# mozilla/mozjpeg

Measured on AMD Instinct MI355X. Metric: Mpixels/s encode (4K RGB q75 trellis) at 1/2/4/8 GPUs; bit-exact vs cjpeg, higher is better.
Workload: dtype u8/int16 (+f32 trellis costs); 1 GPU; 3840x2160 synthetic RGB, q75 4:2:0 baseline, trellis+deringing+optimal Huffman (cjpeg -quality 75 -baseline); config_key=metric, frames_per_encode_call=96, distinct_frames=96, batches_in_flight=2, input=resident in HBM, output=complete JPEG files in HBM, parallelism=images sharded, 1 process per GPU, no collective

## Files before the change

### include/mozjpeg_hip.h

```cpp
#ifndef MOZJPEG_HIP_H
#define MOZJPEG_HIP_H

#include <stddef.h>
#include <stdint.h>

#ifdef __cplusplus
extern "C" {
#endif

#define MJH_MAX_COMPS 4
#define MJH_MAX_SCANS 64

#define MJH_OK            0
#define MJH_EINVAL       -1
#define MJH_EUNSUPPORTED -2
#define MJH_EHIP         -3
#define MJH_ENOMEM       -4
#define MJH_ETOOSMALL    -5

#define MJH_PROFILE_MAX_COMPRESSION 0x5D083AAD
#define MJH_PROFILE_FASTEST         0x2AEA5CB4

typedef struct {
  int comps_in_scan;
// ... 212 lines not shown
  int raw_coefs;
} mjh_decode_opts;
void mjh_decode_opts_defaults(mjh_decode_opts *o);
int mjh_decode_host(mjh_encoder *e, const void *const jpegs[], const size_t sizes[], int n, const mjh_decode_opts *opts);
int mjh_decode_wait(mjh_encoder *e);
int mjh_get_pixels(mjh_encoder *e, int i, void *dst, size_t row_pitch);
int mjh_get_pixels_device(mjh_encoder *e, void **d_base, size_t *row_pitch, size_t *image_stride);
int mjh_get_plane(mjh_encoder *e, int i, int comp, void *dst, size_t row_pitch, int width, int height);
int mjh_get_planes_device(mjh_encoder *e, int comp, void **d_base, size_t *row_pitch, size_t *image_stride, int *width, int *height);
int mjh_get_coefs_device(mjh_encoder *e, int comp, void **d_base, size_t *image_stride, int *blocks_per_row, int *height_in_blocks, int *width_in_blocks);
int mjh_get_coefs(mjh_encoder *e, int i, int comp, void *dst, size_t dst_blocks_per_row);
int mjh_get_coefs_ms(mjh_encoder *e, float *ms);
int mjh_decode_stats(mjh_encoder *e, int *width, int *height, int *pixel_size, float ms[2]);

int mjh_enc_onepass_stats(mjh_encoder *e, int *enabled, unsigned long long *long_blocks, unsigned long long *big_groups);
int mjh_get_dc_path(mjh_encoder *e, int *path);

int mjh_get_jpeg_size(mjh_encoder *e, int i, size_t *size);
int mjh_get_jpeg(mjh_encoder *e, int i, void *dst, size_t cap, size_t *size);
int mjh_get_output_device(mjh_encoder *e, void **d_base, size_t *stride, void **d_sizes);

int mjh_get_scan_table(mjh_encoder *e, int image, int scan, int tblno, uint8_t bits[17], uint8_t vals[256]);

enum {
  MJH_TAP_PLANE = 1,
  MJH_TAP_COEF_UQ = 2,
  MJH_TAP_COEF_Q = 3,
  MJH_TAP_COEF_Q0 = 4,
  MJH_TAP_HUFF_BITS = 5,
  MJH_TAP_HUFF_VALS = 6,
// ... 25 lines not shown
```

### mozjpeg_amd/__init__.py

```python
import ctypes as C
import os

import numpy as np

_HERE = os.path.dirname(os.path.abspath(__file__))
LIB_PATH = os.environ.get("MOZJPEG_AMD_LIB") or os.path.join(_HERE, "libmozjpeg_hip.so")

MAX_COMPS, MAX_SCANS = 4, 64
PROFILE_MAX_COMPRESSION = 0x5D083AAD
PROFILE_FASTEST = 0x2AEA5CB4
COLOR_YCC, COLOR_NONE, COLOR_YCC_IN = 0, 1, 2
CS_GRAYSCALE, CS_RGB, CS_YCBCR = 1, 2, 3
CS_CMYK, CS_YCCK = 4, 5
CS_RGB565 = 16
OK, EINVAL, EUNSUPPORTED, EHIP, ENOMEM, ETOOSMALL = 0, -1, -2, -3, -4, -5
TAP_PLANE, TAP_COEF_UQ, TAP_COEF_Q, TAP_COEF_Q0, TAP_HUFF_BITS, TAP_HUFF_VALS, TAP_PROG_SCAN_US, TAP_LL_COUNTS = 1, 2, 3, 4, 5, 6, 7, 8


class MjhError(RuntimeError):
    def __init__(self, code, msg):
        super().__init__("mozjpeg_hip error %d: %s" % (code, msg))
        self.code = code


# ... 174 lines not shown
            L.mjh_get_pixels_device.argtypes = [C.c_void_p, C.POINTER(C.c_void_p), C.POINTER(C.c_size_t), C.POINTER(C.c_size_t)]
            L.mjh_decode_stats.argtypes = [C.c_void_p, C.POINTER(C.c_int), C.POINTER(C.c_int), C.POINTER(C.c_int), C.POINTER(C.c_float)]
            L.mjh_decode_wait.argtypes = [C.c_void_p]
            L.mjh_get_plane.argtypes = [C.c_void_p, C.c_int, C.c_int, C.c_void_p, C.c_size_t, C.c_int, C.c_int]
            L.mjh_get_planes_device.argtypes = [C.c_void_p, C.c_int, C.POINTER(C.c_void_p), C.POINTER(C.c_size_t), C.POINTER(C.c_size_t),
                                                C.POINTER(C.c_int), C.POINTER(C.c_int)]
            L.mjh_transcode_batch_size.argtypes = [C.c_void_p]
        if hasattr(L, "mjh_get_coefs"):
            L.mjh_get_coefs.argtypes = [C.c_void_p, C.c_int, C.c_int, C.c_void_p, C.c_size_t]
            L.mjh_get_coefs_device.argtypes = [C.c_void_p, C.c_int, C.POINTER(C.c_void_p), C.POINTER(C.c_size_t)] + [C.POINTER(C.c_int)] * 3
            L.mjh_get_coefs_ms.argtypes = [C.c_void_p, C.POINTER(C.c_float)]
        if hasattr(L, "mjh_get_dc_path"):
            L.mjh_get_dc_path.argtypes = [C.c_void_p, C.POINTER(C.c_int)]
        if hasattr(L, "mjh_enc_onepass_stats"):
            L.mjh_enc_onepass_stats.argtypes = [C.c_void_p, C.POINTER(C.c_int), C.POINTER(C.c_ulonglong), C.POINTER(C.c_ulonglong)]
        _lib = L
    return _lib


def _chk(rc):
    if rc != 0:
        raise MjhError(rc, lib().mjh_last_error().decode())


def make_params(width, height, *, quality=75, baseline=False, revert=False, optimize=False,
                notrellis=False, notrellis_dc=False, noovershoot=False, sample=(2, 2), gray=False,
                grayin=False, quant_table=-1, lambda1=None, lambda2=None, restart=None,
                progressive=False, fastcrush=False, precision=8, trellis_loops=1, smooth=0, rgb=False,
                dc_scan_opt=None, dc_ver_weight=None, use_scans_in_trellis=False, trellis_freq_split=0,
                trellis_eob_opt=False, trellis_q_opt=False, arithmetic=False, arith_cond=None, scans=None, gray_sample=None, yccin=False, dct=None,
# ... 657 lines not shown

    def transcode_stats(self):
        a, b, c, ms = C.c_int(), C.c_int(), C.c_int(), (C.c_float * 4)()
        _chk(lib().mjh_transcode_stats(self._h, C.byref(a), C.byref(b), C.byref(c), ms))
        phases = dict(zip(("sync", "prefix", "store", "dc"), [float(x) for x in ms]))
        x = C.c_float()
        if hasattr(lib(), "mjh_get_coefs_ms") and lib().mjh_get_coefs_ms(self._h, C.byref(x)) == OK:
            phases["export"] = float(x.value)
        return dict(subseq=a.value, rounds=b.value, host_syncs=c.value, ms=phases)

    def enc_onepass_stats(self):
        on, a, b = C.c_int(), C.c_ulonglong(), C.c_ulonglong()
        _chk(lib().mjh_enc_onepass_stats(self._h, C.byref(on), C.byref(a), C.byref(b)))
        return dict(enabled=bool(on.value), long_blocks=a.value, big_groups=b.value)

    def dc_path(self):
        v = C.c_int()
        _chk(lib().mjh_get_dc_path(self._h, C.byref(v)))
        return (None, "lane", "dc3", "dc2", "speculative")[v.value]

    def transcode_host(self, files, errors="raise", **transform):
        n = len(files)
        if transform:
            self.set_transform(transform_spec(**transform))
        try:
            self.submit_transcode(files)
            return [self.get_jpeg(i) for i in range(n)]
        except MjhError:
            if errors != "return":
                raise
# ... 160 lines not shown
```

### mozjpeg_amd/csrc/mjh_encoder.cpp

```cpp
#include <hip/hip_runtime.h>

#include <math.h>
#include <stdarg.h>
#include <stdio.h>
#include <stdlib.h>
#include <string.h>

#include <array>
#include <atomic>
#include <condition_variable>
#include <functional>
#include <mutex>
#include <string>
#include <thread>
#include <memory>
#include <chrono>
#include <vector>

#include "../../include/mozjpeg_hip.h"
#include "mjh_internal.h"
#include "mjh_launch.h"
#include "mjh_lossless.h"
#include "mjh_decode.h"
#include "mjh_idct.h"
// ... 290 lines not shown
  void *d_prog_chunks = nullptr;
  int chunks_per_scan = 0;
  MjhProgPE pe{};
  PList pl_trellis[2]{}, pl_phase[4]{}, pl_trellis_c[2][4]{};
  int nphases = 0;
  unsigned *d_pool = nullptr; size_t pool_words = 0;
  uint8_t *d_outpool = nullptr; size_t outpool_bytes = 0;
  uint8_t *d_frame_hdr = nullptr; int frame_hdr_len = 0, file_hdr_len = 0;
  uint16_t *d_len16 = nullptr;
  unsigned *d_off32 = nullptr, *d_sums = nullptr, *d_totals = nullptr, *d_ffsums = nullptr, *d_fftotals = nullptr;
  unsigned *d_stream = nullptr;
  size_t stream_words = 0;
  int enc_onepass = 1;
  unsigned *d_pack = nullptr;
  size_t pack_words = 0;
  unsigned *d_enc_slow = nullptr;
  int chunks = 0, ff_chunks = 0;
  uint8_t *d_out = nullptr;
  size_t out_stride = 0;
  unsigned *d_sizes = nullptr;
  void *d_meta = nullptr;
  uint8_t *d_prefix = nullptr, *d_sos = nullptr;
  int prefix_len = 0, sos_len = 0;
  struct SeqScan { int ncomp; int comp[4]; int sos_off, sos_len; int dht_slots[8], dht_ids[8], ndht; int ri, nseg; };
  std::vector<SeqScan> seq_scans;
  int dht_slots[8] = { 0, 0, 0, 0, 0, 0, 0, 0 }, dht_ids[8] = { 0, 0, 0, 0, 0, 0, 0, 0 }, ndht = 0;
  bool debug_taps = false;
  int dc_chain_v = 1;
  int sof_hv0 = 0;
  bool fdct_div_zero = false;
// ... 545 lines not shown
{
  if (hipStreamSynchronize(a) != hipSuccess || hipStreamSynchronize(b) != hipSuccess) return -1;
  int votes = 0;
  for (int rep = 0; rep < 3; rep++) {
    const auto t0 = std::chrono::steady_clock::now();
    mjh_launch_spin(15000ull, a);
    mjh_launch_spin(15000ull, b);
    if (hipStreamSynchronize(a) != hipSuccess || hipStreamSynchronize(b) != hipSuccess) return -1;
    const double us = std::chrono::duration<double, std::micro>(std::chrono::steady_clock::now() - t0).count();
    votes += us < 240.0;
  }
  return votes >= 2;
}

static thread_local bool g_create_twin = false;
static thread_local int g_twin_onepass = 1;
static thread_local int g_twin_dc_lanes = 0, g_twin_dc_lanes_set = 0;
static thread_local hipStream_t g_twin_avoid[2] = { nullptr, nullptr };

static hipError_t make_streams(mjh_encoder *e)
{
#define STREAMCHK(x) do { const hipError_t r_ = (x); if (r_ != hipSuccess) return r_; } while (0)
  if (e->high_priority_streams) {
    std::vector<hipStream_t> made;
    for (int tries = 0; tries < 12 && !e->side_stream; tries++) {
      hipStream_t c = nullptr;
      STREAMCHK(hipStreamCreateWithFlags(&c, hipStreamNonBlocking));
      made.push_back(c);
      bool free_queue = true;
      for (hipStream_t other : { g_twin_avoid[0], g_twin_avoid[1], e->stream })
// ... 140 lines not shown
  if (const char *v = getenv("MJH_SMALL_BATCH")) e->small_batch = (size_t)atoll(v);
  if (const char *v = getenv("MJH_TRELLIS_CHUNKS")) { e->trellis_chunks = atoi(v); if (e->trellis_chunks < 0 || e->trellis_chunks > 4) e->trellis_chunks = 0; }
  for (int i = 0; i < 4; i++) HIPCHK_E(hipEventCreateWithFlags(&e->ev_chunk[i], hipEventDisableTiming));
  if (const char *v = getenv("MJH_DC_LATE")) { e->dc_late = atoi(v); if (e->dc_late < 0 || e->dc_late > 2) e->dc_late = 1; }
  if (g_create_twin) { e->dc_lanes = g_twin_dc_lanes; e->dc_lanes_set = g_twin_dc_lanes_set; }
  else if (const char *v = getenv("MJH_DC_LANES")) { e->dc_lanes = atoi(v); if (e->dc_lanes < 0) e->dc_lanes = 0; e->dc_lanes_set = 1; }
  e->dc_window_ok = 1;
  for (int i = 0; i < C.ncomp; i++) if (p->quantval[p->quant_tbl_no[i]][0] < 5) e->dc_window_ok = 0;
  if (const char *v = getenv("MJH_DC_SPEC")) e->dc_spec = atoi(v);
  if (const char *v = getenv("MJH_DECODE_SUBSEQ")) { e->dec_subseq = atoi(v); if (e->dec_subseq < 0 || (e->dec_subseq > 0 && e->dec_subseq < 16)) e->dec_subseq = 16; }
  HIPCHK_E(mjh_dmalloc((void **)&e->d_len16, B * (size_t)C.total_mcu_blocks * 2));
  HIPCHK_E(mjh_dmalloc((void **)&e->d_off32, B * (size_t)C.total_mcu_blocks * 4));
  e->chunks = (C.total_mcu_blocks + 2047) / 2048;
  if (g_create_twin) e->enc_onepass = g_twin_onepass;
  else if (const char *v = getenv("MJH_ENC_ONEPASS")) e->enc_onepass = atoi(v) != 0;
  if (e->enc_onepass) {
    e->pack_words = mjh_encode_pack_words(C);
    HIPCHK_E(mjh_dmalloc((void **)&e->d_pack, B * e->pack_words * 4));
    HIPCHK_E(mjh_dmalloc((void **)&e->d_enc_slow, 2 * sizeof(unsigned)));
    HIPCHK_E(hipMemset(e->d_enc_slow, 0, 2 * sizeof(unsigned)));
  }
  size_t words = (size_t)C.total_mcu_blocks * (C.precision == 12 ? 61 : 53) + 64;
  if (C.restart_interval) words += (size_t)(C.mcus_per_row * C.mcu_rows) / C.restart_interval + 1;
  if (words > (size_t)1 << 27) words = (size_t)1 << 27;
  e->stream_words = (words + 63) & ~(size_t)63;
  e->ff_chunks = (int)((e->stream_words + 2047) / 2048);
  HIPCHK_E(mjh_dmalloc((void **)&e->d_sums, B * (size_t)std::max(e->chunks, mjh_encode_segments(C)) * sizeof(unsigned)));
  HIPCHK_E(mjh_dmalloc((void **)&e->d_ffsums, B * e->ff_chunks * sizeof(unsigned)));
  HIPCHK_E(mjh_dmalloc((void **)&e->d_totals, B * sizeof(unsigned)));
  HIPCHK_E(mjh_dmalloc((void **)&e->d_fftotals, B * sizeof(unsigned)));
// ... 818 lines not shown
        int slots[8], ns = 0;
        for (int j = 0; j < q.ncomp; j++) {
          bool have_d = false, have_a = false;
          for (int t = 0; t < ns; t++) { have_d = have_d || slots[t] == v_dc[j]; have_a = have_a || slots[t] == v_ac[j]; }
          if (!have_d) slots[ns++] = v_dc[j];
          if (!have_a) slots[ns++] = v_ac[j];
        }
        mjh_launch_gen_tables(e->d_tabs, spi, slots, ns, n, s);
      }
      pr.mark("header");
      mjh_launch_header(si == 0 ? e->d_prefix : nullptr, si == 0 ? e->prefix_len : 0, e->d_sos + q.sos_off, q.sos_len, e->d_tabs, spi, q.dht_slots, q.dht_ids, q.ndht,
                        p.compress_profile != MJH_PROFILE_FASTEST, e->d_out, e->out_stride, e->d_meta, n, s, si == 0 ? nullptr : e->d_sizes);
      pr.mark("huff_encode");
      mjh_launch_encode(V, e->d_q, nzm, e->d_tabs, spi, v_dc, v_ac, e->d_len16, e->d_off32, e->d_sums, e->chunks, e->d_totals,
                        e->d_stream, e->stream_words, e->d_meta, e->d_seg_x, e->d_seg_E, e->d_seg_sums, e->d_seg_totals, e->d_mpos, q.nseg, n, s,
                        e->d_pack, e->pack_words, e->d_enc_slow);
      pr.mark("byte_stuff");
      mjh_launch_stuff(e->d_stream, e->stream_words, e->d_totals, e->d_ffsums, e->ff_chunks, e->d_fftotals, e->d_out, e->out_stride,
                       e->d_meta, e->d_sizes, e->d_mpos, q.nseg, n, s);
    }
  } else {
    if (p.optimize_coding) {
      pr.mark("stats_ac(final)");
      mjh_launch_stats_ac(C, e->d_q, nzm, e->d_tabs, spi, fin_ac, 1, n, s);
      if (!final_dc_counted) {
        pr.mark("stats_dc(final)");
        mjh_launch_stats_dc(C, e->d_q, e->d_tabs, spi, fin_dc, 1, zero4, n, s);
      }
      if (join_late) {
        pr.mark("join(trellis_dc)");
        HIPCHK(hipStreamWaitEvent(s, e->ev_join, 0));
      }
      pr.mark("gen_tables(final)");
      mjh_launch_gen_tables(e->d_tabs, spi, e->dht_slots, e->ndht, n, s);
    }
    if (before_output) HIPCHK(hipStreamWaitEvent(s, before_output, 0));
    pr.mark("header");
    mjh_launch_header(e->d_prefix, e->prefix_len, e->d_sos, e->sos_len, e->d_tabs, spi, e->dht_slots, e->dht_ids, e->ndht,
                      p.compress_profile != MJH_PROFILE_FASTEST, e->d_out, e->out_stride, e->d_meta, n, s);
    pr.mark("huff_encode");
    mjh_launch_encode(C, e->d_q, nzm, e->d_tabs, spi, fin_dc, fin_ac, e->d_len16, e->d_off32, e->d_sums, e->chunks, e->d_totals,
                      e->d_stream, e->stream_words, e->d_meta, e->d_seg_x, e->d_seg_E, e->d_seg_sums, e->d_seg_totals, e->d_mpos, e->nseg, n, s,
                      e->d_pack, e->pack_words, e->d_enc_slow);
    if (if_mode == 2) { HIPCHK(hipEventRecord(e->ev_done, s)); e->ev_done_set = true; }
    pr.mark("byte_stuff");
    mjh_launch_stuff(e->d_stream, e->stream_words, e->d_totals, e->d_ffsums, e->ff_chunks, e->d_fftotals, e->d_out, e->out_stride,
                     e->d_meta, e->d_sizes, e->d_mpos, e->nseg, n, s);
  }
  if (ext_qopt) {
    pr.mark("trellis_q_opt(DQT)");
    mjh_launch_qopt_fix(e->d_quant, e->d_out, e->out_stride, e->d_sizes, e->file_hdr_len, e->prefix_len - (10 + 3 * C.ncomp), e->dqt_tabs, e->dqt_ntab,
                        p.compress_profile != MJH_PROFILE_FASTEST, !e->progressive && C.precision == 8 && e->tbl_le1, n, s);
  }
  pr.mark(nullptr);
  pr.finish();
  if (peer && !(if_mode == 2 && e->ev_done_set)) { HIPCHK(hipEventRecord(e->ev_done, s)); e->ev_done_set = true; }
  HIPCHK(hipGetLastError());
  return MJH_OK;
// ... 3 lines not shown

static mjh_encoder *cur(mjh_encoder *e) { return e && e->last ? e->last : e; }

extern "C" int mjh_set_inflight(mjh_encoder *e, int batches)
{
  if (!e || batches < 1 || batches > 2) return fail(MJH_EINVAL, "batches in flight: 1 or 2");
  e->inflight = batches;
  return MJH_OK;
}

static int make_twin(mjh_encoder *e)
{
  mjh_encoder *t = nullptr;
  g_create_twin = true;
  g_twin_onepass = e->enc_onepass;
  g_twin_dc_lanes = e->dc_lanes; g_twin_dc_lanes_set = e->dc_lanes_set;
  g_twin_avoid[0] = e->stream; g_twin_avoid[1] = e->side_stream;
  const int rc = mjh_encoder_create(&e->p_created, e->max_batch, e->device, &t);
  g_create_twin = false;
  if (rc) return rc;
  t->owner = e;
  t->inflight = 1;
  t->profiling = e->profiling; t->prof_focus_name = e->prof_focus_name; t->prof_focus = e->prof_focus;
  e->twin = t;
  return MJH_OK;
}

static int wait_pending_pack(mjh_encoder *e, hipStream_t s)
{
  if (e->res_buf >= 0 && !e->res_waited[e->res_buf]) HIPCHK(hipStreamWaitEvent(s, e->ev_packed[e->res_buf], 0));
// ... 1968 lines not shown
  if (enabled) *enabled = e->enc_onepass;
  unsigned long long a = 0, b = 0;
  for (mjh_encoder *x : { e, e->twin }) {
    if (!x || !x->d_enc_slow) continue;
    unsigned h[2] = { 0, 0 };
    HIPCHK(hipSetDevice(x->device));
    HIPCHK(hipDeviceSynchronize());
    HIPCHK(hipMemcpy(h, x->d_enc_slow, sizeof(h), hipMemcpyDeviceToHost));
    a += h[0]; b += h[1];
  }
  if (long_blocks) *long_blocks = a;
  if (big_groups) *big_groups = b;
  return MJH_OK;
}

extern "C" int mjh_encoder_sync(mjh_encoder *e)
{
  if (!e) return fail(MJH_EINVAL, "null encoder");
  HIPCHK(hipSetDevice(e->device));
  HIPCHK(hipStreamSynchronize(e->last_stream ? e->last_stream : e->stream));
  if (e->twin) HIPCHK(hipStreamSynchronize(e->twin->last_stream ? e->twin->last_stream : e->twin->stream));
  return guard_verify();
}

static int fetch_sizes(mjh_encoder *e)
{
  if (e->sizes_valid) return MJH_OK;
  if (e->res_buf >= 0) {
    int rc = wait_results(e, e->res_buf);
    if (rc) return rc;
// ... 487 lines not shown
```

### mozjpeg_amd/csrc/mjh_kernels.hip

```cpp
#include <hip/hip_runtime.h>
#include <stdio.h>
#include <stdlib.h>
#include <stdint.h>
#include <type_traits>
#include <stdlib.h>
#include "mjh_internal.h"
#include "mjh_device.h"

#define WAVE 64

struct ZZTab { int v[64]; };
static constexpr ZZTab make_zz() {
  ZZTab t{};
  const int z[64] = {
    0,  1,  8, 16,  9,  2,  3, 10, 17, 24, 32, 25, 18, 11,  4,  5,
    12, 19, 26, 33, 40, 48, 41, 34, 27, 20, 13,  6,  7, 14, 21, 28,
    35, 42, 49, 56, 57, 50, 43, 36, 29, 22, 15, 23, 30, 37, 44, 51,
    58, 59, 52, 45, 38, 31, 39, 46, 53, 60, 61, 54, 47, 55, 62, 63 };
  for (int i = 0; i < 64; i++) t.v[i] = z[i];
  return t;
}
static constexpr ZZTab kZZ = make_zz();

#define FIXC(x) ((int)((x) * 65536.0 + 0.5))
// ... 647 lines not shown
  __syncthreads();
  const int c4 = (lane & 7) * 4;
#pragma unroll
  for (int i = 0; i < 8; i++) {
    const int b = i * 8 + (lane >> 3);
    const unsigned *t = tile + b * 33 + c4;
    if (d0 + b < ndst) *reinterpret_cast<uint4 *>(out + (size_t)(d0 + b) * 128 + (size_t)c4 * 4) = make_uint4(t[0], t[1], t[2], t[3]);
  }
}
template <class F>
__device__ __forceinline__ void for_each_nonzero(const int16_t *__restrict__ qb, size_t kstride, unsigned long long mask, bool active, F &&f)
{
  const int n = active ? __popcll(mask) : 0;
#pragma unroll 1
  for (int base = 0; base < 63; base += 8) {
    if (__builtin_amdgcn_ballot_w64(base < n) == 0ull) break;
    int v[8];
#pragma unroll
    for (int j = 0; j < 8; j++) v[j] = (base + j < n) ? (int)qb[(size_t)(base + j + 1) * kstride] : 0;
#pragma unroll
    for (int j = 0; j < 8; j++)
      if (base + j < n) {
        const int pos = __builtin_ctzll(mask);
        mask &= mask - 1ull;
        f(pos, v[j]);
      }
  }
}

#define STATS_AC_ITER 4
// ... 1092 lines not shown
  __device__ __forceinline__ MarkerCursor(const unsigned *m, int nmark) : mpos(m), n(nmark), idx(-1) {}
  __device__ __forceinline__ bool at(unsigned bytepos)
  {
    if (idx < 0) {
      int lo = 0, hi = n;
      while (lo < hi) { const int mid = (lo + hi) >> 1; if (mpos[mid] < bytepos) lo = mid + 1; else hi = mid; }
      idx = lo;
    }
    while (idx < n && mpos[idx] < bytepos) idx++;
    return idx < n && mpos[idx] == bytepos;
  }
};

#define ENCW_WIN 4096

template <bool COMPACT, class W>
__device__ __forceinline__ void enc_write_block(const MjhConst &C, const MjhComp &cc, W &bw, const unsigned *s_ac, const unsigned *s_dc,
                                                const int16_t *__restrict__ q, const unsigned long long *__restrict__ nzmask_img, int r, int c,
                                                int *dc_nbits = nullptr)
{
  const int dc = q[dc_source_block(cc, r, c)];
  int pr, pc, pred = 0;
  if (mcu_prev_block(C, cc, r, c, pr, pc)) pred = q[dc_source_block(cc, pr, pc)];
  {
    const int df = dc - pred;
    const int a = df < 0 ? -df : df;
    const int nb = bitlen((unsigned)a);
    if (dc_nbits) *dc_nbits = nb;
    const unsigned e = s_dc[nb];
    bw.put(e & 0xFFFF, (int)(e >> 16));
// ... 100 lines not shown
      bw.flush();
    };
    if (window) { BitSink<true> bw; bw.init(s_win, fo - (w0 << 5)); emit(bw, w0 << 5); }
    else { BitSink<false> bw; bw.init(g, fo); emit(bw, 0u); }
  }
  __syncthreads();
  if (window)
    for (unsigned i = tid; i < nw; i += 256) {
      const unsigned v = s_win[i];
      if (v == 0u) continue;
      if (i == 0u || i == nw - 1u) atomicOr(&g[w0 + i], v);
      else g[w0 + i] = v;
    }
}

#define ENCP_DEPTH 8
#define ENCP_WIN 2048

__device__ __forceinline__ void enc_load_tables(unsigned (*s_ac)[256], unsigned (*s_dc)[32], const MjhConst &C, const MjhHuffTable *__restrict__ tabs_img,
                                                const int4 &dc_slot_of_comp, const int4 &ac_slot_of_comp)
{
  const int tid = threadIdx.x;
  for (int ci = 0; ci < C.ncomp; ci++) {
    const int dslot = ci == 0 ? dc_slot_of_comp.x : ci == 1 ? dc_slot_of_comp.y : ci == 2 ? dc_slot_of_comp.z : dc_slot_of_comp.w;
    const int aslot = ci == 0 ? ac_slot_of_comp.x : ci == 1 ? ac_slot_of_comp.y : ci == 2 ? ac_slot_of_comp.z : ac_slot_of_comp.w;
    const MjhHuffTable *TD = tabs_img + dslot;
    const MjhHuffTable *TA = tabs_img + aslot;
    s_ac[ci][tid] = ((unsigned)TA->ehufsi[tid] << 16) | TA->ehufco[tid];
    if (tid < 32) s_dc[ci][tid] = tid < 16 ? ((unsigned)TD->ehufsi[tid] << 16) | TD->ehufco[tid] : 0u;
  }
}

__device__ __forceinline__ int enc_scan_position(const MjhConst &C, int p, int &r, int &c)
{
  const int mcu = p / C.blocks_per_mcu, bi = p - mcu * C.blocks_per_mcu;
  int comp = 0;
  for (int ci = 1; ci < C.ncomp; ci++) if (bi >= C.c[ci].mcu_blk0) comp = ci;
  const int h = C.c[comp].h, v = C.c[comp].v;
  const int local = bi - C.c[comp].mcu_blk0, yi = local / h, xi = local - yi * h;
  const int mrow = mcu / C.mcus_per_row, mcol = mcu - mrow * C.mcus_per_row;
  r = mrow * v + yi;
  c = mcol * h + xi;
  return comp;
}

template <bool COMPACT>
__global__ void __launch_bounds__(256)
k_enc_write_pack(MjhConst C, const int16_t *__restrict__ coef_q, const unsigned long long *__restrict__ nzmask, const MjhHuffTable *__restrict__ tabs,
                 int slots_per_image, int4 dc_slot_of_comp, int4 ac_slot_of_comp,
                 unsigned *__restrict__ pack, size_t pack_words_per_image, unsigned *__restrict__ sums, int segs_per_image,
                 MjhImageMeta *__restrict__ meta, unsigned *__restrict__ slow)
{
  __shared__ unsigned s_ac[MJH_MAXC][256];
  __shared__ unsigned s_dc[MJH_MAXC][32];
  __shared__ unsigned s_stage[ENCP_DEPTH * 256];
  __shared__ uint4 s_win4[ENCP_WIN / 4];
  __shared__ unsigned sh[8];
  unsigned *s_win = reinterpret_cast<unsigned *>(s_win4);
  const int img = blockIdx.y, tid = threadIdx.x;
  const int N = C.total_mcu_blocks, p = blockIdx.x * 256 + tid;
  enc_load_tables(s_ac, s_dc, C, tabs + (size_t)img * slots_per_image, dc_slot_of_comp, ac_slot_of_comp);
  for (int i = tid; i < ENCP_WIN / 4; i += 256) s_win4[i] = make_uint4(0u, 0u, 0u, 0u);
  __syncthreads();
  int r = 0, c = 0;
  const int comp = enc_scan_position(C, p < N ? p : 0, r, c);
  const MjhComp cc = C.c[comp];
  const int16_t *q = coef_q + (size_t)img * C.coefs_per_image + cc.coef_off;
  const unsigned long long *nzi = COMPACT ? nzmask + (size_t)img * C.total_real_blocks : nullptr;
  unsigned bits = 0;
  if (p < N) {
    MJH_DIVERGENT_SCOPE;
    StageSink<ENCP_DEPTH, 256> bw;
    bw.init(s_stage + tid);
    int nb = 0;
    enc_write_block<COMPACT>(C, cc, bw, s_ac[comp], s_dc[comp], q, nzi, r, c, &nb);
    bw.flush();
    bits = bw.bitpos();
    if (nb > (C.precision == 12 ? 15 : 11)) meta[img].bad_coef = 1u;
  }
  unsigned tot;
  const unsigned ex = block_excl_scan_256_1b(bits, sh, 0, &tot);
  if (tid == 0) sums[(size_t)img * segs_per_image + blockIdx.x] = tot;
  const unsigned nw = (tot + 31u) >> 5;
  if (nw > (unsigned)ENCP_WIN) {
    if (tid == 0) atomicAdd(&slow[1], 1u);
    return;
  }
  if (bits > ENCP_DEPTH * 32u) {
    MJH_DIVERGENT_SCOPE;
    atomicAdd(&slow[0], 1u);
    BitSink<true, false> bw;
    bw.init(s_win, ex);
    enc_write_block<COMPACT>(C, cc, bw, s_ac[comp], s_dc[comp], q, nzi, r, c);
    bw.flush();
  } else {
    const unsigned s = ex & 31u, w0 = ex >> 5, nsw = (bits + 31u) >> 5, ndw = (s + bits + 31u) >> 5;
    unsigned prev = 0u;
    for (unsigned k = 0; k < ndw; k++) {
      const unsigned cur = k < nsw ? s_stage[k * 256 + tid] : 0u;
      const unsigned v = funnel_shift(prev, cur, s);
      if (v) atomicOr(&s_win[w0 + k], v);
      prev = cur;
    }
  }
  __syncthreads();
  unsigned *g = pack + (size_t)img * pack_words_per_image + (size_t)blockIdx.x * ENCP_WIN;
  for (unsigned i = tid; i < nw; i += 256) g[i] = s_win[i];
}

__global__ void __launch_bounds__(256)
k_enc_write_place(const unsigned *__restrict__ pack, size_t pack_words_per_image, const unsigned *__restrict__ sums, int segs_per_image,
                  const unsigned *__restrict__ totals, unsigned *__restrict__ stream, size_t stream_words_per_image)
{
  const int img = blockIdx.y, lane = threadIdx.x & 63;
  const int seg = blockIdx.x * 4 + (threadIdx.x >> 6);
  if (seg >= segs_per_image) return;
  const unsigned total = totals[img];
  if (total == 0xFFFFFFFFu) return;
  const unsigned *sm = sums + (size_t)img * segs_per_image;
  const unsigned base = sm[seg], len = (seg + 1 < segs_per_image ? sm[seg + 1] : total) - base;
  const unsigned nsw = (len + 31u) >> 5;
  if (nsw > (unsigned)ENCP_WIN) return;
// ... 545 lines not shown
    return MJH_DC_PATH_LANE;
  }
  dim3 grid((chain1 - chain0 + 3) / 4, n);
  if (window_ok && C.delta_dc_weight <= 0.0f) {
    hipLaunchKernelGGL(k_trellis_dc3, grid, dim3(64), 0, s, C, Q, (const int16_t *)uq, (int16_t *)q, tabs, spi, make_int4(dc_slot[0], dc_slot[1], dc_slot[2], dc_slot[3]), lambda, (uint8_t *)back, chain0, chain1);
    return MJH_DC_PATH_DC3;
  }
  hipLaunchKernelGGL(k_trellis_dc2, grid, dim3(64), 0, s, C, Q, (const int16_t *)uq, (int16_t *)q, tabs, spi, make_int4(dc_slot[0], dc_slot[1], dc_slot[2], dc_slot[3]), lambda, (uint8_t *)back, chain0, chain1);
  return MJH_DC_PATH_DC2;
}

void mjh_launch_encode(const MjhConst &C, const void *q, const unsigned long long *nzmask, const MjhHuffTable *tabs, int spi, const int dc_slot[4], const int ac_slot[4],
                       void *len16, void *off32, unsigned *sums, int chunks_per_image, unsigned *totals,
                       unsigned *stream, size_t stream_words_per_image, void *meta,
                       unsigned *seg_x, unsigned *seg_E, unsigned *seg_sums, unsigned *seg_totals, unsigned *mpos, int nseg,
                       int n, hipStream_t s, unsigned *pack, size_t pack_words_per_image, unsigned *slow)
{
  const int4 ds = make_int4(dc_slot[0], dc_slot[1], dc_slot[2], dc_slot[3]);
  const int4 as = make_int4(ac_slot[0], ac_slot[1], ac_slot[2], ac_slot[3]);
  if (pack && C.restart_interval == 0) {
    const int segs = mjh_encode_segments(C);
    dim3 gridp(segs, n);
    if (nzmask) hipLaunchKernelGGL((k_enc_write_pack<true>), gridp, dim3(256), 0, s, C, (const int16_t *)q, nzmask, tabs, spi, ds, as, pack, pack_words_per_image, sums, segs,
                                   (MjhImageMeta *)meta, slow);
    else hipLaunchKernelGGL((k_enc_write_pack<false>), gridp, dim3(256), 0, s, C, (const int16_t *)q, nzmask, tabs, spi, ds, as, pack, pack_words_per_image, sums, segs,
                            (MjhImageMeta *)meta, slow);
    hipLaunchKernelGGL(k_scan_sums, dim3(n), dim3(256), 0, s, sums, segs, totals, (const unsigned *)nullptr);
    hipLaunchKernelGGL(k_zero_stream, dim3(64, n), dim3(256), 0, s, stream, stream_words_per_image, (const unsigned *)totals, (const unsigned *)nullptr);
    hipLaunchKernelGGL(k_enc_write_place, dim3((segs + 3) / 4, n), dim3(256), 0, s, (const unsigned *)pack, pack_words_per_image, (const unsigned *)sums, segs,
                       (const unsigned *)totals, stream, stream_words_per_image);
    dim3 gridb((segs + 255) / 256, n);
    if (nzmask) hipLaunchKernelGGL((k_enc_write_big<true>), gridb, dim3(256), 0, s, C, (const int16_t *)q, nzmask, tabs, spi, ds, as, (const unsigned *)sums, segs,
                                   (const unsigned *)totals, stream, stream_words_per_image);
    else hipLaunchKernelGGL((k_enc_write_big<false>), gridb, dim3(256), 0, s, C, (const int16_t *)q, nzmask, tabs, spi, ds, as, (const unsigned *)sums, segs,
                            (const unsigned *)totals, stream, stream_words_per_image);
    hipLaunchKernelGGL(k_finish_bits, dim3((n + 63) / 64), dim3(64), 0, s, totals, (const unsigned *)nullptr, stream, stream_words_per_image, (MjhImageMeta *)meta, n);
    return;
  }
  dim3 grid((max_padblk(C) + 255) / 256, C.ncomp, n);
  if (nzmask) hipLaunchKernelGGL((k_enc_len<true>), grid, dim3(256), 0, s, C, (const int16_t *)q, nzmask, tabs, spi, ds, as, (uint16_t *)len16, (MjhImageMeta *)meta);
  else hipLaunchKernelGGL((k_enc_len<false>), grid, dim3(256), 0, s, C, (const int16_t *)q, nzmask, tabs, spi, ds, as, (uint16_t *)len16, (MjhImageMeta *)meta);
// ... 59 lines not shown
```

### mozjpeg_amd/csrc/mjh_launch.h

```cpp
#ifndef MJH_LAUNCH_H
#define MJH_LAUNCH_H
#include <hip/hip_runtime.h>
#include "mjh_internal.h"

void mjh_launch_import_coefs(const MjhConst &C, const MjhCoefSrc &S, void *coef_q, void *meta, int n, hipStream_t s);
void mjh_launch_export_coefs(const MjhConst &C, const MjhCoefDst &D, const void *coef_q, const unsigned *status, int n, hipStream_t s);
void mjh_launch_import_planes(const MjhConst &C, const MjhPlaneSrc &S, void *planes, int n, hipStream_t s);
void mjh_launch_color(const MjhConst &C, const void *pix, size_t row_pitch, size_t img_stride, void *planes, int n, hipStream_t s);
void mjh_launch_dct(const MjhConst &C, const MjhQuant *Q, const void *planes, void *uq, void *q, float *lambda,
                    MjhHuffTable *stat_tabs, int spi, const int stat_slot[4], uint8_t *nq8, int n, hipStream_t s, int fastdiv = 0, int ifast = 0);
void mjh_launch_stats_ac(const MjhConst &C, const void *q, const unsigned long long *nzmask, MjhHuffTable *tabs, int spi, const int slot[4], int count_dummies, int n, hipStream_t s);
void mjh_launch_stats_dc(const MjhConst &C, const void *q, MjhHuffTable *tabs, int spi, const int slot[4], int mcu_order, const int comp_restart[4], int n, hipStream_t s);
void mjh_launch_gen_tables(MjhHuffTable *tabs, int spi, const int *slots, int nslots, int n, hipStream_t s);
void mjh_launch_trellis_ac(const MjhConst &C, const MjhQuant *Q, const void *uq, void *q, MjhHuffTable *tabs, int spi, const int ac_slot[4], const float *lambda,
                           unsigned *worklist, unsigned *worklist2, void *dense, unsigned dense_cap, int variant,
                           int Ss, int Se, void *eob_cost, int *eob_has, unsigned long long *nzmask, int qstride, int n, hipStream_t s,
                           uint8_t *nq8 = nullptr, int v3_passes = 0, int fastdiv = 0, hipEvent_t after_first_tier = nullptr, hipEvent_t after_first_tier2 = nullptr,
                           int chunks = 1, hipStream_t side = nullptr, hipEvent_t *ev_chunk = nullptr, int count_mask = 0);
void mjh_launch_trellis_eob_chain(const MjhConst &C, void *q, const MjhHuffTable *tabs, int spi, const int ac_slot[4], const void *eob_cost, const int *eob_has,
                                  int Ss, int Se, int n, hipStream_t s);
void mjh_launch_qopt_accumulate(const MjhConst &C, const void *uq, const void *q, void *sums, int n, hipStream_t s);
void mjh_launch_qopt_update(void *sums, MjhQuant *Q, int n, hipStream_t s);
void mjh_launch_qopt_fix(const MjhQuant *Q, void *out, size_t out_stride, unsigned *sizes, int dqt_start, int sof_off, const int *tabs, int ntab,
                         int multi, int baseline_capable, int n, hipStream_t s);
enum { MJH_DC_PATH_NONE = 0, MJH_DC_PATH_LANE = 1, MJH_DC_PATH_DC3 = 2, MJH_DC_PATH_DC2 = 3, MJH_DC_PATH_SPEC = 4 };
bool mjh_trellis_dc_lanes_ok(const MjhConst &C, int window_ok, int n, int lanes_min);
int mjh_launch_trellis_dc(const MjhConst &C, const MjhQuant *Q, const void *uq, void *q, const MjhHuffTable *tabs, int spi, const int dc_slot[4], const float *lambda, void *back, int n, hipStream_t s,
                          int window_ok = 0, int chain0 = 0, int chain1 = -1, int lanes_min = 0);
void mjh_launch_encode(const MjhConst &C, const void *q, const unsigned long long *nzmask, const MjhHuffTable *tabs, int spi, const int dc_slot[4], const int ac_slot[4],
                       void *len16, void *off32, unsigned *sums, int chunks_per_image, unsigned *totals,
                       unsigned *stream, size_t stream_words_per_image, void *meta,
                       unsigned *seg_x, unsigned *seg_E, unsigned *seg_sums, unsigned *seg_totals, unsigned *mpos, int nseg,
                       int n, hipStream_t s, unsigned *pack = nullptr, size_t pack_words_per_image = 0, unsigned *slow = nullptr);
int mjh_encode_segments(const MjhConst &C);
size_t mjh_encode_pack_words(const MjhConst &C);
void mjh_launch_header(const void *prefix, int prefix_len, const void *sos, int sos_len, const MjhHuffTable *tabs, int spi,
                       const int dht_slots[8], const int dht_ids[8], int ndht, int multi_dht, void *out, size_t out_stride, void *meta, int n, hipStream_t s, const unsigned *append_sizes = nullptr);
void mjh_launch_finish_bits(unsigned *totals, unsigned *stream, size_t stream_words_per_image, void *meta, int n, hipStream_t s);
void mjh_launch_stuff(const unsigned *stream, size_t stream_words_per_image, const unsigned *totals, unsigned *ffsums, int ff_chunks_per_image,
                      unsigned *ff_totals, void *out, size_t out_stride, void *meta, unsigned *sizes, const unsigned *mpos, int nseg, int n, hipStream_t s);
void mjh_launch_pack_results(const void *out, size_t out_stride, const unsigned *sizes, const void *meta, const void *prog_ctl, int n,
                             void *dst, size_t cap, void *table, hipStream_t s);
void mjh_launch_pack_results_spliced(const void *out, size_t out_stride, const unsigned *sizes, const void *meta, const void *prog_ctl, int n,
                                     const MjhSpliceFile *files, const MjhSpliceRun *runs, const void *tc, const void *icc, unsigned icc_len, unsigned hdr,
                                     void *dst, size_t cap, void *table, hipStream_t s);
void mjh_launch_spin(unsigned long long ticks_100mhz, hipStream_t s);
void mjh_launch_gen_tables_list(MjhHuffTable *tabs, int spi, const int *d_slots, int nslots, int n, hipStream_t s);
void mjh_launch_prog_reset(void *ctl, int nscans, int n, hipStream_t s);
// ... 25 lines not shown
```

Measured before the change: 159,100 Mpixels/s.

## Persist pack-encode blocks across segment groups with prefetch and division-free scan positions

Measured after the change: 164,300 Mpixels/s (median of 6 runs). 1.03x the previous value.

```diff
diff --git a/include/mozjpeg_hip.h b/include/mozjpeg_hip.h
--- a/include/mozjpeg_hip.h
+++ b/include/mozjpeg_hip.h
@@ -250,6 +250,7 @@
 int mjh_decode_stats(mjh_encoder *e, int *width, int *height, int *pixel_size, float ms[2]);
 
 int mjh_enc_onepass_stats(mjh_encoder *e, int *enabled, unsigned long long *long_blocks, unsigned long long *big_groups);
+int mjh_enc_pack_groups(mjh_encoder *e, int *groups, int *twin_groups);
 int mjh_get_dc_path(mjh_encoder *e, int *path);
 
 int mjh_get_jpeg_size(mjh_encoder *e, int i, size_t *size);
diff --git a/mozjpeg_amd/__init__.py b/mozjpeg_amd/__init__.py
--- a/mozjpeg_amd/__init__.py
+++ b/mozjpeg_amd/__init__.py
@@ -212,6 +212,9 @@
             L.mjh_get_dc_path.argtypes = [C.c_void_p, C.POINTER(C.c_int)]
         if hasattr(L, "mjh_enc_onepass_stats"):
             L.mjh_enc_onepass_stats.argtypes = [C.c_void_p, C.POINTER(C.c_int), C.POINTER(C.c_ulonglong), C.POINTER(C.c_ulonglong)]
+        if hasattr(L, "mjh_enc_pack_groups"):
+            L.mjh_enc_pack_groups.argtypes = [C.c_void_p, C.POINTER(C.c_int), C.POINTER(C.c_int)]
+            L.mjh_enc_scan_positions.argtypes = [C.c_int] + [C.POINTER(C.c_int)] * 4 + [C.c_int, C.POINTER(C.c_int), C.c_int, C.POINTER(C.c_int)]
         _lib = L
     return _lib
 
@@ -899,6 +902,11 @@
         _chk(lib().mjh_enc_onepass_stats(self._h, C.byref(on), C.byref(a), C.byref(b)))
         return dict(enabled=bool(on.value), long_blocks=a.value, big_groups=b.value)
 
+    def enc_pack_groups(self):
+        g, t = C.c_int(), C.c_int()
+        _chk(lib().mjh_enc_pack_groups(self._h, C.byref(g), C.byref(t)))
+        return g.value, (None if t.value < 0 else t.value)
+
     def dc_path(self):
         v = C.c_int()
         _chk(lib().mjh_get_dc_path(self._h, C.byref(v)))
diff --git a/mozjpeg_amd/csrc/mjh_encoder.cpp b/mozjpeg_amd/csrc/mjh_encoder.cpp
--- a/mozjpeg_amd/csrc/mjh_encoder.cpp
+++ b/mozjpeg_amd/csrc/mjh_encoder.cpp
@@ -328,6 +328,7 @@
   int enc_onepass = 1;
   unsigned *d_pack = nullptr;
   size_t pack_words = 0;
+  int encp_groups = MJH_ENCP_GROUPS_DEFAULT;
   unsigned *d_enc_slow = nullptr;
   int chunks = 0, ff_chunks = 0;
   uint8_t *d_out = nullptr;
@@ -903,6 +904,7 @@
 }
 
 static thread_local bool g_create_twin = false;
+static thread_local int g_twin_encp_groups = MJH_ENCP_GROUPS_DEFAULT;
 static thread_local int g_twin_onepass = 1;
 static thread_local int g_twin_dc_lanes = 0, g_twin_dc_lanes_set = 0;
 static thread_local hipStream_t g_twin_avoid[2] = { nullptr, nullptr };
@@ -1073,6 +1075,8 @@
   e->chunks = (C.total_mcu_blocks + 2047) / 2048;
   if (g_create_twin) e->enc_onepass = g_twin_onepass;
   else if (const char *v = getenv("MJH_ENC_ONEPASS")) e->enc_onepass = atoi(v) != 0;
+  if (g_create_twin) e->encp_groups = g_twin_encp_groups;
+  else if (const char *v = getenv("MJH_ENCP_GROUPS")) { e->encp_groups = atoi(v); if (e->encp_groups < 1 || e->encp_groups > 64) e->encp_groups = MJH_ENCP_GROUPS_DEFAULT; }
   if (e->enc_onepass) {
     e->pack_words = mjh_encode_pack_words(C);
     HIPCHK_E(mjh_dmalloc((void **)&e->d_pack, B * e->pack_words * 4));
@@ -1921,7 +1925,7 @@
       pr.mark("huff_encode");
       mjh_launch_encode(V, e->d_q, nzm, e->d_tabs, spi, v_dc, v_ac, e->d_len16, e->d_off32, e->d_sums, e->chunks, e->d_totals,
                         e->d_stream, e->stream_words, e->d_meta, e->d_seg_x, e->d_seg_E, e->d_seg_sums, e->d_seg_totals, e->d_mpos, q.nseg, n, s,
-                        e->d_pack, e->pack_words, e->d_enc_slow);
+                        e->d_pack, e->pack_words, e->d_enc_slow, e->encp_groups);
       pr.mark("byte_stuff");
       mjh_launch_stuff(e->d_stream, e->stream_words, e->d_totals, e->d_ffsums, e->ff_chunks, e->d_fftotals, e->d_out, e->out_stride,
                        e->d_meta, e->d_sizes, e->d_mpos, q.nseg, n, s);
@@ -1948,7 +1952,7 @@
     pr.mark("huff_encode");
     mjh_launch_encode(C, e->d_q, nzm, e->d_tabs, spi, fin_dc, fin_ac, e->d_len16, e->d_off32, e->d_sums, e->chunks, e->d_totals,
                       e->d_stream, e->stream_words, e->d_meta, e->d_seg_x, e->d_seg_E, e->d_seg_sums, e->d_seg_totals, e->d_mpos, e->nseg, n, s,
-                      e->d_pack, e->pack_words, e->d_enc_slow);
+                      e->d_pack, e->pack_words, e->d_enc_slow, e->encp_groups);
     if (if_mode == 2) { HIPCHK(hipEventRecord(e->ev_done, s)); e->ev_done_set = true; }
     pr.mark("byte_stuff");
     mjh_launch_stuff(e->d_stream, e->stream_words, e->d_totals, e->d_ffsums, e->ff_chunks, e->d_fftotals, e->d_out, e->out_stride,
@@ -1982,6 +1986,7 @@
   mjh_encoder *t = nullptr;
   g_create_twin = true;
   g_twin_onepass = e->enc_onepass;
+  g_twin_encp_groups = e->encp_groups;
   g_twin_dc_lanes = e->dc_lanes; g_twin_dc_lanes_set = e->dc_lanes_set;
   g_twin_avoid[0] = e->stream; g_twin_avoid[1] = e->side_stream;
   const int rc = mjh_encoder_create(&e->p_created, e->max_batch, e->device, &t);
@@ -3980,6 +3985,14 @@
   return MJH_OK;
 }
 
+extern "C" int mjh_enc_pack_groups(mjh_encoder *e, int *groups, int *twin_groups)
+{
+  if (!e) return fail(MJH_EINVAL, "null encoder");
+  if (groups) *groups = e->encp_groups;
+  if (twin_groups) *twin_groups = e->twin ? e->twin->encp_groups : -1;
+  return MJH_OK;
+}
+
 extern "C" int mjh_encoder_sync(mjh_encoder *e)
 {
   if (!e) return fail(MJH_EINVAL, "null encoder");
diff --git a/mozjpeg_amd/csrc/mjh_kernels.hip b/mozjpeg_amd/csrc/mjh_kernels.hip
--- a/mozjpeg_amd/csrc/mjh_kernels.hip
+++ b/mozjpeg_amd/csrc/mjh_kernels.hip
@@ -685,6 +685,33 @@
   const int n = active ? __popcll(mask) : 0;
 #pragma unroll 1
   for (int base = 0; base < 63; base += 8) {
+    if (__builtin_amdgcn_ballot_w64(base < n) == 0ull) break;
+    int v[8];
+#pragma unroll
+    for (int j = 0; j < 8; j++) v[j] = (base + j < n) ? (int)qb[(size_t)(base + j + 1) * kstride] : 0;
+#pragma unroll
+    for (int j = 0; j < 8; j++)
+      if (base + j < n) {
+        const int pos = __builtin_ctzll(mask);
+        mask &= mask - 1ull;
+        f(pos, v[j]);
+      }
+  }
+}
+
+template <class F>
+__device__ __forceinline__ void for_each_nonzero_from(const int *v0, const int16_t *__restrict__ qb, size_t kstride, unsigned long long mask, bool active, F &&f)
+{
+  const int n = active ? __popcll(mask) : 0;
+#pragma unroll
+  for (int j = 0; j < 8; j++)
+    if (j < n) {
+      const int pos = __builtin_ctzll(mask);
+      mask &= mask - 1ull;
+      f(pos, v0[j]);
+    }
+#pragma unroll 1
+  for (int base = 8; base < 63; base += 8) {
     if (__builtin_amdgcn_ballot_w64(base < n) == 0ull) break;
     int v[8];
 #pragma unroll
@@ -1807,6 +1834,62 @@
 
 #define ENCW_WIN 4096
 
+template <class W>
+__device__ __forceinline__ void enc_put_dc(W &bw, const unsigned *s_dc, int df, int *dc_nbits)
+{
+  const int a = df < 0 ? -df : df;
+  const int nb = bitlen((unsigned)a);
+  if (dc_nbits) *dc_nbits = nb;
+  const unsigned e = s_dc[nb];
+  bw.put(e & 0xFFFF, (int)(e >> 16));
+  if (nb) bw.put((unsigned)(df < 0 ? df - 1 : df), nb);
+}
+
+template <bool COMPACT, class W>
+__device__ __forceinline__ void enc_put_ac(int kstride, W &bw, const unsigned *s_ac, const int16_t *__restrict__ q, unsigned long long m, bool real, int b,
+                                           const int *v0 = nullptr)
+{
+  if (COMPACT) {
+    int prev = 0;
+    auto sym = [&](int pos, int v) {
+      int run = pos - prev - 1;
+      prev = pos;
+      while (run > 15) { const unsigned e = s_ac[0xF0]; bw.put(e & 0xFFFF, (int)(e >> 16)); run -= 16; }
+      const int a = v < 0 ? -v : v;
+      const int nbv = bitlen((unsigned)a);
+      const unsigned e = s_ac[(run << 4) + nbv];
+      bw.put_sym(e, (unsigned)(v < 0 ? v - 1 : v), nbv);
+    };
+    if (v0) for_each_nonzero_from(v0, q + b, (size_t)kstride, m, real, sym);
+    else for_each_nonzero(q + b, (size_t)kstride, m, real, sym);
+    if (!real || prev < 63) { const unsigned e = s_ac[0]; bw.put(e & 0xFFFF, (int)(e >> 16)); }
+  } else {
+    int x[64];
+#pragma unroll
+    for (int k = 1; k < 64; k++) x[k] = q[(size_t)k * kstride + b];
+    if (real) {
+      int run = 0;
+#pragma unroll
+      for (int k = 1; k < 64; k++) {
+        const int v = x[k];
+        if (v == 0) run++;
+        else {
+          while (run > 15) { const unsigned e = s_ac[0xF0]; bw.put(e & 0xFFFF, (int)(e >> 16)); run -= 16; }
+          const int a = v < 0 ? -v : v;
+          const int nb = bitlen((unsigned)a);
+          const unsigned e = s_ac[(run << 4) + nb];
+          bw.put_sym(e, (unsigned)(v < 0 ? v - 1 : v), nb);
+          run = 0;
+        }
+      }
+      if (run > 0) { const unsigned e = s_ac[0]; bw.put(e & 0xFFFF, (int)(e >> 16)); }
+    } else {
+      const unsigned e = s_ac[0];
+      bw.put(e & 0xFFFF, (int)(e >> 16));
+    }
+  }
+}
+
 template <bool COMPACT, class W>
 __device__ __forceinline__ void enc_write_block(const MjhConst &C, const MjhComp &cc, W &bw, const unsigned *s_ac, const unsigned *s_dc,
                                                 const int16_t *__restrict__ q, const unsigned long long *__restrict__ nzmask_img, int r, int c,
@@ -1937,7 +2020,14 @@
     }
 }
 
+#ifndef ENCP_DEPTH
 #define ENCP_DEPTH 8
+#endif
+#ifdef ENCP_MIN_WAVES
+#define ENCP_BOUNDS __launch_bounds__(256, ENCP_MIN_WAVES)
+#else
+#define ENCP_BOUNDS __launch_bounds__(256)
+#endif
 #define ENCP_WIN 2048
 
 __device__ __forceinline__ void enc_load_tables(unsigned (*s_ac)[256], unsigned (*s_dc)[32], const MjhConst &C, const MjhHuffTable *__restrict__ tabs_img,
@@ -1967,68 +2057,191 @@
   return comp;
 }
 
+__host__ __device__ __forceinline__ int udiv_m31(int n, unsigned m, unsigned s)
+{
+  return (int)((unsigned)(((unsigned long long)((unsigned)n << 1) * m) >> 32) >> s);
+}
+
+static void mjh_enc_div_magic(unsigned d, unsigned *m, unsigned *s)
+{
+  unsigned sh = 0;
+  while ((1u << sh) < d) sh++;
+  *m = (unsigned)((((unsigned long long)1 << (31 + sh)) + d - 1) / d);
+  *s = sh;
+}
+
+struct EncComp { int h, v, wib, hib, mcu_blk0, kstride; long long coef_off, blk_off; };
+__host__ __device__ __forceinline__ EncComp enc_comp(const MjhComp &m)
+{
+  EncComp e;
+  e.h = m.h; e.v = m.v; e.wib = m.wib; e.hib = m.hib; e.mcu_blk0 = m.mcu_blk0; e.kstride = m.kstride; e.coef_off = m.coef_off; e.blk_off = m.blk_off;
+  return e;
+}
+
+__host__ __device__ __forceinline__ int enc_dc_source(const EncComp &cc, int r, int c, int mcol)
+{
+  if (r >= cc.hib) { c = mcol * cc.h + cc.h - 1; r = cc.hib - 1; }
+  if (c > cc.wib - 1) c = cc.wib - 1;
+  return r * cc.wib + c;
+}
+
+__host__ __device__ __forceinline__ int enc_scan_position_nodiv(const MjhConst &C, const EncComp *cs, const uint4 &dv, int p, int &r, int &c, int &dc_blk, int &pred_blk)
+{
+  const int mcu = udiv_m31(p, dv.x, dv.y), bi = p - mcu * C.blocks_per_mcu;
+  int comp = 0;
+  for (int ci = 1; ci < C.ncomp; ci++) if (bi >= C.c[ci].mcu_blk0) comp = ci;
+  const EncComp cc = cs[comp];
+  const int h = cc.h, v = cc.v;
+  const int local = bi - cc.mcu_blk0;
+  const int yi = (local * (int)((0x10162040u >> (8 * (h - 1))) & 0xFFu)) >> 6, xi = local - yi * h;
+  const int mrow = udiv_m31(mcu, dv.z, dv.w), mcol = mcu - mrow * C.mcus_per_row;
+  r = mrow * v + yi;
+  c = mcol * h + xi;
+  dc_blk = enc_dc_source(cc, r, c, mcol);
+  int pr = r, pc = c - 1, pmcol = mcol;
+  bool has = true;
+  if (xi == 0) {
+    if (yi > 0) { pr = r - 1; pc = c + h - 1; }
+    else if (mcu == 0) has = false;
+    else {
+      const bool wrap = mcol == 0;
+      pmcol = wrap ? C.mcus_per_row - 1 : mcol - 1;
+      pr = (wrap ? mrow - 1 : mrow) * v + v - 1;
+      pc = pmcol * h + h - 1;
+    }
+  }
+  pred_blk = has ? enc_dc_source(cc, pr, pc, pmcol) : -1;
+  return comp;
+}
+
+extern "C" int mjh_enc_scan_positions(int ncomp, const int *h, const int *v, const int *wib, const int *hib, int mcus_per_row,
+                                      const int *p, int np, int *out)
+{
+  if (ncomp < 1 || ncomp > MJH_MAXC || mcus_per_row < 1) return -1;
+  MjhConst C{};
+  C.ncomp = ncomp;
+  C.mcus_per_row = mcus_per_row;
+  for (int i = 0; i < ncomp; i++) {
+    if (h[i] < 1 || h[i] > 4 || v[i] < 1 || v[i] > 4) return -1;
+    C.c[i].h = h[i]; C.c[i].v = v[i]; C.c[i].wib = wib[i]; C.c[i].hib = hib[i];
+    C.c[i].mcu_blk0 = C.blocks_per_mcu;
+    C.blocks_per_mcu += h[i] * v[i];
+  }
+  EncComp cs[MJH_MAXC];
+  for (int i = 0; i < ncomp; i++) cs[i] = enc_comp(C.c[i]);
+  uint4 dv;
+  mjh_enc_div_magic((unsigned)C.blocks_per_mcu, &dv.x, &dv.y);
+  mjh_enc_div_magic((unsigned)C.mcus_per_row, &dv.z, &dv.w);
+  for (int i = 0; i < np; i++) {
+    int *o = out + 5 * (size_t)i;
+    o[0] = enc_scan_position_nodiv(C, cs, dv, p[i], o[1], o[2], o[3], o[4]);
+  }
+  return 0;
+}
+
+#ifndef ENCP_AHEAD
+#define ENCP_AHEAD 1
+#endif
+#ifndef ENCP_EARLY
+#define ENCP_EARLY 1
+#endif
 template <bool COMPACT>
-__global__ void __launch_bounds__(256)
+__global__ void ENCP_BOUNDS
 k_enc_write_pack(MjhConst C, const int16_t *__restrict__ coef_q, const unsigned long long *__restrict__ nzmask, const MjhHuffTable *__restrict__ tabs,
                  int slots_per_image, int4 dc_slot_of_comp, int4 ac_slot_of_comp,
                  unsigned *__restrict__ pack, size_t pack_words_per_image, unsigned *__restrict__ sums, int segs_per_image,
-                 MjhImageMeta *__restrict__ meta, unsigned *__restrict__ slow)
+                 MjhImageMeta *__restrict__ meta, unsigned *__restrict__ slow, int groups, uint4 dv)
 {
   __shared__ unsigned s_ac[MJH_MAXC][256];
   __shared__ unsigned s_dc[MJH_MAXC][32];
   __shared__ unsigned s_stage[ENCP_DEPTH * 256];
   __shared__ uint4 s_win4[ENCP_WIN / 4];
   __shared__ unsigned sh[8];
+  __shared__ EncComp s_cc[MJH_MAXC];
   unsigned *s_win = reinterpret_cast<unsigned *>(s_win4);
+  constexpr bool AHEAD = COMPACT && ENCP_AHEAD;
   const int img = blockIdx.y, tid = threadIdx.x;
-  const int N = C.total_mcu_blocks, p = blockIdx.x * 256 + tid;
+  const int N = C.total_mcu_blocks;
+  if (tid < C.ncomp) s_cc[tid] = enc_comp(C.c[tid]);
+  if (AHEAD && ENCP_EARLY) __syncthreads();
+  const int16_t *qimg = coef_q + (size_t)img * C.coefs_per_image;
+  const unsigned long long *nzi = COMPACT ? nzmask + (size_t)img * C.total_real_blocks : nullptr;
+  const int max_nb = C.precision == 12 ? 15 : 11;
+  const int seg0 = blockIdx.x * groups, seg1 = min(seg0 + groups, segs_per_image);
+  struct Pos { int comp, b, df, kstride; bool real; const int16_t *q; unsigned long long m; int v0[8]; };
+  auto fetch = [&](int seg, Pos &P) {
+    const int p = seg * 256 + tid;
+    int r, c, dcb, pdb;
+    P.comp = enc_scan_position_nodiv(C, s_cc, dv, p < N ? p : 0, r, c, dcb, pdb);
+    const EncComp cc = s_cc[P.comp];
+    P.q = qimg + cc.coef_off;
+    P.real = r < cc.hib && c < cc.wib;
+    P.b = P.real ? r * cc.wib + c : 0;
+    P.kstride = cc.kstride;
+    P.m = 0ull;
+    if (COMPACT) P.m = nzi[cc.blk_off + P.b];
+    if (AHEAD) {
+#pragma unroll
+      for (int j = 0; j < 8; j++) P.v0[j] = (int)P.q[(size_t)(j + 1) * cc.kstride + P.b];
+    }
+    const int dc = P.q[dcb], pred = P.q[pdb < 0 ? dcb : pdb];
+    P.df = dc - (pdb < 0 ? 0 : pred);
+  };
+  Pos P;
+  if (AHEAD && ENCP_EARLY) fetch(seg0, P);
   enc_load_tables(s_ac, s_dc, C, tabs + (size_t)img * slots_per_image, dc_slot_of_comp, ac_slot_of_comp);
   for (int i = tid; i < ENCP_WIN / 4; i += 256) s_win4[i] = make_uint4(0u, 0u, 0u, 0u);
   __syncthreads();
-  int r = 0, c = 0;
-  const int comp = enc_scan_position(C, p < N ? p : 0, r, c);
-  const MjhComp cc = C.c[comp];
-  const int16_t *q = coef_q + (size_t)img * C.coefs_per_image + cc.coef_off;
-  const unsigned long long *nzi = COMPACT ? nzmask + (size_t)img * C.total_real_blocks : nullptr;
-  unsigned bits = 0;
-  if (p < N) {
-    MJH_DIVERGENT_SCOPE;
-    StageSink<ENCP_DEPTH, 256> bw;
-    bw.init(s_stage + tid);
-    int nb = 0;
-    enc_write_block<COMPACT>(C, cc, bw, s_ac[comp], s_dc[comp], q, nzi, r, c, &nb);
-    bw.flush();
-    bits = bw.bitpos();
-    if (nb > (C.precision == 12 ? 15 : 11)) meta[img].bad_coef = 1u;
-  }
-  unsigned tot;
-  const unsigned ex = block_excl_scan_256_1b(bits, sh, 0, &tot);
-  if (tid == 0) sums[(size_t)img * segs_per_image + blockIdx.x] = tot;
-  const unsigned nw = (tot + 31u) >> 5;
-  if (nw > (unsigned)ENCP_WIN) {
-    if (tid == 0) atomicAdd(&slow[1], 1u);
-    return;
-  }
-  if (bits > ENCP_DEPTH * 32u) {
-    MJH_DIVERGENT_SCOPE;
-    atomicAdd(&slow[0], 1u);
-    BitSink<true, false> bw;
-    bw.init(s_win, ex);
-    enc_write_block<COMPACT>(C, cc, bw, s_ac[comp], s_dc[comp], q, nzi, r, c);
-    bw.flush();
-  } else {
-    const unsigned s = ex & 31u, w0 = ex >> 5, nsw = (bits + 31u) >> 5, ndw = (s + bits + 31u) >> 5;
-    unsigned prev = 0u;
-    for (unsigned k = 0; k < ndw; k++) {
-      const unsigned cur = k < nsw ? s_stage[k * 256 + tid] : 0u;
-      const unsigned v = funnel_shift(prev, cur, s);
-      if (v) atomicOr(&s_win[w0 + k], v);
-      prev = cur;
-    }
-  }
-  __syncthreads();
-  unsigned *g = pack + (size_t)img * pack_words_per_image + (size_t)blockIdx.x * ENCP_WIN;
-  for (unsigned i = tid; i < nw; i += 256) g[i] = s_win[i];
+  if (AHEAD && !ENCP_EARLY) fetch(seg0, P);
+#pragma unroll 1
+  for (int seg = seg0; seg < seg1; seg++) {
+    if (!AHEAD) fetch(seg, P);
+    const int p = seg * 256 + tid, comp = P.comp, kstride = P.kstride;
+    unsigned bits = 0;
+    if (p < N) {
+      MJH_DIVERGENT_SCOPE;
+      StageSink<ENCP_DEPTH, 256> bw;
+      bw.init(s_stage + tid);
+      int nb = 0;
+      enc_put_dc(bw, s_dc[comp], P.df, &nb);
+      enc_put_ac<COMPACT>(kstride, bw, s_ac[comp], P.q, P.m, P.real, P.b, AHEAD ? P.v0 : nullptr);
+      bw.flush();
+      bits = bw.bitpos();
+      if (nb > max_nb) meta[img].bad_coef = 1u;
+    }
+    if (AHEAD && seg + 1 < seg1) fetch(seg + 1, P);
+    unsigned tot;
+    const unsigned ex = block_excl_scan_256_1b(bits, sh, (seg - seg0) & 1, &tot);
+    if (tid == 0) sums[(size_t)img * segs_per_image + seg] = tot;
+    const unsigned nw = (tot + 31u) >> 5;
+    if (nw > (unsigned)ENCP_WIN) {
+      if (tid == 0) atomicAdd(&slow[1], 1u);
+      continue;
+    }
+    if (bits > ENCP_DEPTH * 32u) {
+      MJH_DIVERGENT_SCOPE;
+      atomicAdd(&slow[0], 1u);
+      Pos Q;
+      fetch(seg, Q);
+      BitSink<true, false> bw;
+      bw.init(s_win, ex);
+      enc_put_dc(bw, s_dc[comp], Q.df, nullptr);
+      enc_put_ac<COMPACT>(Q.kstride, bw, s_ac[comp], Q.q, Q.m, Q.real, Q.b);
+      bw.flush();
+    } else {
+      const unsigned s = ex & 31u, w0 = ex >> 5, nsw = (bits + 31u) >> 5, ndw = (s + bits + 31u) >> 5;
+      unsigned prev = 0u;
+      for (unsigned k = 0; k < ndw; k++) {
+        const unsigned cw = k < nsw ? s_stage[k * 256 + tid] : 0u;
+        const unsigned v = funnel_shift(prev, cw, s);
+        if (v) atomicOr(&s_win[w0 + k], v);
+        prev = cw;
+      }
+    }
+    __syncthreads();
+    uint4 *g = reinterpret_cast<uint4 *>(pack + (size_t)img * pack_words_per_image + (size_t)seg * ENCP_WIN);
+    for (unsigned i = tid; i < (nw + 3u) >> 2; i += 256) { g[i] = s_win4[i]; s_win4[i] = make_uint4(0u, 0u, 0u, 0u); }
+  }
 }
 
 __global__ void __launch_bounds__(256)
@@ -2604,17 +2817,21 @@
                        void *len16, void *off32, unsigned *sums, int chunks_per_image, unsigned *totals,
                        unsigned *stream, size_t stream_words_per_image, void *meta,
                        unsigned *seg_x, unsigned *seg_E, unsigned *seg_sums, unsigned *seg_totals, unsigned *mpos, int nseg,
-                       int n, hipStream_t s, unsigned *pack, size_t pack_words_per_image, unsigned *slow)
+                       int n, hipStream_t s, unsigned *pack, size_t pack_words_per_image, unsigned *slow, int pack_groups)
 {
   const int4 ds = make_int4(dc_slot[0], dc_slot[1], dc_slot[2], dc_slot[3]);
   const int4 as = make_int4(ac_slot[0], ac_slot[1], ac_slot[2], ac_slot[3]);
   if (pack && C.restart_interval == 0) {
     const int segs = mjh_encode_segments(C);
-    dim3 gridp(segs, n);
+    const int G = pack_groups < 1 ? 1 : pack_groups;
+    dim3 gridp((segs + G - 1) / G, n);
+    uint4 dv;
+    mjh_enc_div_magic((unsigned)C.blocks_per_mcu, &dv.x, &dv.y);
+    mjh_enc_div_magic((unsigned)C.mcus_per_row, &dv.z, &dv.w);
     if (nzmask) hipLaunchKernelGGL((k_enc_write_pack<true>), gridp, dim3(256), 0, s, C, (const int16_t *)q, nzmask, tabs, spi, ds, as, pack, pack_words_per_image, sums, segs,
-                                   (MjhImageMeta *)meta, slow);
+                                   (MjhImageMeta *)meta, slow, G, dv);
     else hipLaunchKernelGGL((k_enc_write_pack<false>), gridp, dim3(256), 0, s, C, (const int16_t *)q, nzmask, tabs, spi, ds, as, pack, pack_words_per_image, sums, segs,
-                            (MjhImageMeta *)meta, slow);
+                            (MjhImageMeta *)meta, slow, G, dv);
     hipLaunchKernelGGL(k_scan_sums, dim3(n), dim3(256), 0, s, sums, segs, totals, (const unsigned *)nullptr);
     hipLaunchKernelGGL(k_zero_stream, dim3(64, n), dim3(256), 0, s, stream, stream_words_per_image, (const unsigned *)totals, (const unsigned *)nullptr);
     hipLaunchKernelGGL(k_enc_write_place, dim3((segs + 3) / 4, n), dim3(256), 0, s, (const unsigned *)pack, pack_words_per_image, (const unsigned *)sums, segs,
diff --git a/mozjpeg_amd/csrc/mjh_launch.h b/mozjpeg_amd/csrc/mjh_launch.h
--- a/mozjpeg_amd/csrc/mjh_launch.h
+++ b/mozjpeg_amd/csrc/mjh_launch.h
@@ -31,7 +31,8 @@
                        void *len16, void *off32, unsigned *sums, int chunks_per_image, unsigned *totals,
                        unsigned *stream, size_t stream_words_per_image, void *meta,
                        unsigned *seg_x, unsigned *seg_E, unsigned *seg_sums, unsigned *seg_totals, unsigned *mpos, int nseg,
-                       int n, hipStream_t s, unsigned *pack = nullptr, size_t pack_words_per_image = 0, unsigned *slow = nullptr);
+                       int n, hipStream_t s, unsigned *pack = nullptr, size_t pack_words_per_image = 0, unsigned *slow = nullptr, int pack_groups = 1);
+#define MJH_ENCP_GROUPS_DEFAULT 4
 int mjh_encode_segments(const MjhConst &C);
 size_t mjh_encode_pack_words(const MjhConst &C);
 void mjh_launch_header(const void *prefix, int prefix_len, const void *sos, int sos_len, const MjhHuffTable *tabs, int spi,
```
